# marict/nnue-vision

Hardware: AMD Instinct MI355X
Metric: NNUE training images/sec (full step: fwd+bwd+clip+SGD) (higher is better)
Workload: dtype f32; 1 GPU; c2: NNUE 32x32 grid 10x10x8 F=800 -> 1024/128/32 -> 10, batch 512/GPU, SGD m0.9 wd2e-4 clip1.0; global_batch=512, parallelism=dp1, launch=hipGraph, steps_per_graph=26, max_active_features=453

## Files before the change

nnue-vision_amd/csrc/classifier_kernels.hip:

```cpp
#include <type_traits>
#include <cstdlib>
#include <cstring>

#include "common.h"
#include "small_wgrad.h"

namespace {

using f32x4 = __attribute__((ext_vector_type(4))) float;

__device__ __forceinline__ float act_fn(float z, float clip) {
  const float r = z <= 0.0f ? 0.0f : z;
  return (clip > 0.0f && r > clip) ? clip : r;
}
__device__ __forceinline__ float gate_fn(float d, float h, float clip) {
  if (clip > 0.0f) return (h > 0.0f && h < clip) ? d : 0.0f;
  return h <= 0.0f ? 0.0f : d;
}

__device__ __forceinline__ float l0_at(const float* __restrict__ xr, int k, int half, int pairwise) {
  if (!pairwise) return xr[k];
  return k < half ? xr[k] * xr[k + half] : xr[k - half];
}

// ... 674 lines not shown
      const float* __restrict__ wr = w3 + (size_t)c * L3;
      if constexpr (VEC) {
        int k = 4 * part4;
        if (c0 == 0) {
#pragma unroll
          for (int i = 0; i < kPre3; ++i) {
            const int kk = 4 * (part4 + 4 * i);
            if (kk < L3) z = tail_dot4(w3v[i], *reinterpret_cast<const float4*>(h2s + kk), z);
          }
          k += 16 * kPre3;
        }
        for (; k < L3; k += 16) z = tail_dot4(*reinterpret_cast<const float4*>(wr + k), *reinterpret_cast<const float4*>(h2s + k), z);
      } else {
        for (int k = part4; k < L3; k += 4) z = fmaf(wr[k], h2s[k], z);
      }
    }
    z += __shfl_xor(z, 1);
    z += __shfl_xor(z, 2);
    if (c < C && part4 == 0) {
      z += (VEC && c0 == 0) ? b3v : b3[c];
      lgs[c] = z;
      logits[(size_t)b * C + c] = z;
    }
  }
  __syncthreads();
  float mx = -INFINITY, se = 0.f;
  if (C <= 64) {
    const int lane = tid & 63;
    const float v[1] = {lane < C ? lgs[lane] : -INFINITY};
    float m1[1], s1[1];
    ce_wave_stats<1>(v, lane < C, m1, s1);
    mx = m1[0];
    se = s1[0];
  } else {
    for (int c = tid; c < C; c += NT) mx = fmaxf(mx, lgs[c]);
    mx = block_reduce_nt<NT>(mx, true, red);
    for (int c = tid; c < C; c += NT) se += expf(lgs[c] - mx);
    se = block_reduce_nt<NT>(se, false, red);
  }
  const bool ok = y >= 0 && y < C;
  if (tid == 0) sample_loss[b] = ok ? nnue_ce_sample_loss(mx, lgs[y], se) : 0.0f;
  const float inv = 1.0f / se;
  __syncthreads();
  for (int c = tid; c < C; c += NT) {
    const float g = ok ? ce_dlogit(lgs[c], mx, inv, c == y, scale_over_b) : 0.0f;
    lgs[c] = g;
    d_logits[(size_t)b * C + c] = g;
  }
  __syncthreads();
  for (int j0 = 0; j0 < L3; j0 += 32) {
    const int j = j0 + (tid & 31), cp = tid >> 5;
    part_s[cp][tid & 31] = j < L3 ? dz2_slice<S>(lgs, w3 + j, cp, C, L3) : 0.0f;
    __syncthreads();
    if (cp == 0 && j < L3) {
      float q[S];
#pragma unroll
      for (int i = 0; i < S; ++i) q[i] = part_s[i][tid];
      const float v = gate_fn(slice_tree<S>(q), h2s[j], clip);
      dz2s[j] = v;
      d_z2[(size_t)b * L3 + j] = v;
    }
    __syncthreads();
  }
  for (int k = tid; k < L2; k += NT) {
    float s = 0.f;
    int j = 0;
    for (; j + 16 <= L3; j += 16) {
      float w[16];
#pragma unroll
      for (int u = 0; u < 16; ++u) w[u] = w2[(size_t)(j + u) * L2 + k];
#pragma unroll
      for (int u = 0; u < 16; ++u) s = fmaf(dz2s[j + u], w[u], s);
    }
    for (; j < L3; ++j) s = fmaf(dz2s[j], w2[(size_t)j * L2 + k], s);
    const float v = gate_fn(s, h1s[k], clip);
    d_z1[(size_t)b * L2 + k] = v;
    if (d_z1_g) d_z1_g[(size_t)g * L2 + k] = v;
  }
  __syncthreads();
}

constexpr int kTdxRows = 16, kTdxThreads = 512, kTdxMaxC = 64;

template <int S>
__device__ __forceinline__ float dz2_slice_small(const float* dl, const float* w3j, int cp, int C, int L3) {
  float s0 = 0.f, s1 = 0.f, s2 = 0.f, s3 = 0.f;
  int c = cp;
  for (int m = 0, mu = C > 3 * S ? (C - 3 * S + 4 * S - 1) / (4 * S) : 0; m < mu; ++m) {
    const bool act = c + 3 * S < C;
    const int cc = act ? c : 0;
    const float f0 = fmaf(dl[cc], w3j[(size_t)cc * L3], s0), f1 = fmaf(dl[cc + S], w3j[(size_t)(cc + S) * L3], s1);
    const float f2 = fmaf(dl[cc + 2 * S], w3j[(size_t)(cc + 2 * S) * L3], s2), f3 = fmaf(dl[cc + 3 * S], w3j[(size_t)(cc + 3 * S) * L3], s3);
    s0 = act ? f0 : s0; s1 = act ? f1 : s1; s2 = act ? f2 : s2; s3 = act ? f3 : s3;
    c = act ? c + 4 * S : c;
  }
#pragma unroll
  for (int t = 0; t < 3; ++t) {
    const bool act = c + S * t < C;
    const int cc = act ? c + S * t : 0;
    const float f = fmaf(dl[cc], w3j[(size_t)cc * L3], s0);
    s0 = act ? f : s0;
  }
  return (s0 + s1) + (s2 + s3);
}

template <int L2, int L3>
__global__ __launch_bounds__(kTdxThreads) void tail_dx_train_kernel(
    const float* __restrict__ part, int ksplit, const float* __restrict__ b1, const float* __restrict__ w2,
    const float* __restrict__ b2, const float* __restrict__ w3, const float* __restrict__ b3, float clip,
    const int64_t* __restrict__ labels, float scale_over_b, int B, int C, float* __restrict__ h1, float* __restrict__ h2,
    float* __restrict__ logits, float* __restrict__ sample_loss, float* __restrict__ d_logits, float* __restrict__ d_z1,
    float* __restrict__ d_z2, const float* __restrict__ x, const float* __restrict__ w1, int L1, float* __restrict__ d_x,
    int m_tiles, int n_cg) {
  constexpr int T = kTdxRows, NT = kTdxThreads, NWAVE = NT / 64;
  constexpr int NI = T * L2 / 4 / NT;
  constexpr int NCH = L2 / (16 * kBwxKC);
  constexpr int RP = NT / 4 / L3;
  static_assert(NI >= 1 && NI * NT * 4 == T * L2 && NT % L2 == 0 && L3 % 16 == 0 && (NT / 4) % L3 == 0 && T % RP == 0,
                "tail_dx_train_kernel: unsupported layer widths");
  __shared__ float4 w2s4[L3 * L2 / 4];
  __shared__ float4 w3s4[kTdxMaxC * L3 / 4];
  __shared__ __attribute__((aligned(16))) float h1s[T][L2];
  __shared__ __attribute__((aligned(16))) float dz1s[T][L2];
  __shared__ __attribute__((aligned(16))) float h2s[T][L3];
  __shared__ float dz2s[T][L3];
  __shared__ float ps[T][4][L3];
  __shared__ float lgs[T][kTdxMaxC];
  __shared__ float b2s[L3], b3s[kTdxMaxC];
  __shared__ int64_t ys[T];
  __shared__ f32x4 xch[NWAVE][64];
  const float* w2s = reinterpret_cast<const float*>(w2s4);
  const float* w3s = reinterpret_cast<const float*>(w3s4);

  const int blk = blockIdx.x, slot = blk >> 3;
  const int mt = (slot / n_cg) * 8 + (blk & 7), cg = slot % n_cg;
  if (mt >= m_tiles) return;
  const bool writer = cg == 0;
  const int row0 = mt * T;
  const int tid = threadIdx.x;

  const int wave = __builtin_amdgcn_readfirstlane(tid >> 6);
  const int lane = tid & 63;
  const int r = lane & 15, q = lane >> 4;
  const int half = L1 / 2;
  const int hi = wave & 1;
  const int c0 = (cg * (NWAVE / 2) + (wave >> 1)) * 16, c1 = c0 + half, cm = hi ? c1 : c0;
  int orows[4];
#pragma unroll
  for (int e = 0; e < 4; ++e) orows[e] = row0 + 4 * q + e;
  float bw[NCH][kBwxKC][4];
#pragma unroll
  for (int n = 0; n < NCH; ++n) bwx_load_b_tile(bw[n], w1, n * 16 * kBwxKC, L1, L2, cm, r, q);
  float xv[4];
#pragma unroll
  for (int e = 0; e < 4; ++e) xv[e] = x[(size_t)min(orows[e], B - 1) * L1 + (hi ? c0 : c1) + r];

  constexpr int NW2 = L3 * L2 / 4 / NT;
  constexpr int NW3 = kTdxMaxC * L3 / 4 / NT;
  static_assert(NW2 >= 1 && NW2 * NT * 4 == L3 * L2 && NW3 >= 1 && NW3 * NT * 4 == kTdxMaxC * L3, "tail_dx_train_kernel: staging shape");
  float4 w2v[NW2], w3v[NW3];
#pragma unroll
  for (int i = 0; i < NW2; ++i) w2v[i] = reinterpret_cast<const float4*>(w2)[tid + NT * i];
  const int n_w3 = C * L3 / 4;
#pragma unroll
  for (int i = 0; i < NW3; ++i) w3v[i] = reinterpret_cast<const float4*>(w3)[min(tid + NT * i, n_w3 - 1)];
  const float b2v = b2[tid % L3];
  const float b3v = b3[min(tid, C - 1)];
  const int64_t yv = labels[min(row0 + (tid % T), B - 1)];
  int srow[NI], scol[NI];
  float4 z4[NI];
  const float* prow[NI];
#pragma unroll
  for (int i = 0; i < NI; ++i) {
    const int f = tid + NT * i;
    srow[i] = f / (L2 / 4);
    scol[i] = 4 * (f % (L2 / 4));
    prow[i] = part + (size_t)min(row0 + srow[i], B - 1) * L2 + scol[i];
    z4[i] = make_float4(b1[scol[i]], b1[scol[i] + 1], b1[scol[i] + 2], b1[scol[i] + 3]);
  }
  const size_t slab = (size_t)B * L2;
  auto load_batch = [&](int s0, float4 (&v)[NI][16]) {
#pragma unroll
    for (int i = 0; i < NI; ++i)
#pragma unroll
      for (int u = 0; u < 16; ++u) v[i][u] = *reinterpret_cast<const float4*>(prow[i] + (size_t)min(s0 + u, ksplit - 1) * slab);
  };
  auto sum_batch = [&](int s0, const float4 (&v)[NI][16]) {
#pragma unroll
    for (int i = 0; i < NI; ++i)
#pragma unroll
      for (int u = 0; u < 16; ++u) {
        const bool add = s0 + u < ksplit;
        z4[i].x = add ? z4[i].x + v[i][u].x : z4[i].x;
        z4[i].y = add ? z4[i].y + v[i][u].y : z4[i].y;
        z4[i].z = add ? z4[i].z + v[i][u].z : z4[i].z;
        z4[i].w = add ? z4[i].w + v[i][u].w : z4[i].w;
      }
  };
  {
    float4 v[NI][16];
    load_batch(0, v);
#pragma unroll
    for (int i = 0; i < NW2; ++i) w2s4[tid + NT * i] = w2v[i];
#pragma unroll
    for (int i = 0; i < NW3; ++i)
      if (tid + NT * i < n_w3) w3s4[tid + NT * i] = w3v[i];
    if (tid < L3) b2s[tid] = b2v;
    if (tid < C) b3s[tid] = b3v;
    if (tid < T) ys[tid] = row0 + tid < B ? yv : -1;
    sum_batch(0, v);
  }
  for (int s0 = 16; s0 < ksplit; s0 += 16) {
    float4 v[NI][16];
    load_batch(s0, v);
    sum_batch(s0, v);
  }

#pragma unroll
  for (int i = 0; i < NI; ++i) {
    float4 h;
    h.x = act_fn(z4[i].x, clip); h.y = act_fn(z4[i].y, clip); h.z = act_fn(z4[i].z, clip); h.w = act_fn(z4[i].w, clip);
    *reinterpret_cast<float4*>(&h1s[srow[i]][scol[i]]) = h;
    if (writer && row0 + srow[i] < B) *reinterpret_cast<float4*>(h1 + (size_t)(row0 + srow[i]) * L2 + scol[i]) = h;
  }
  __syncthreads();

  const int part4 = tid & 3, og = tid >> 2;
  {
    const int j = og % L3;
    float4 wf[L2 / 16];
#pragma unroll
    for (int m = 0; m < L2 / 16; ++m) wf[m] = w2s4[(j * L2 + 4 * part4 + 16 * m) / 4];
    const float bj = b2s[j];
#pragma unroll
    for (int it = 0; it < T / RP; ++it) {
      const int rr = og / L3 + RP * it;
      float z = 0.f;
#pragma unroll
      for (int m = 0; m < L2 / 16; ++m) z = tail_dot4(wf[m], *reinterpret_cast<const float4*>(&h1s[rr][4 * part4 + 16 * m]), z);
      z += lane_xor<1>(z);
      z += lane_xor<2>(z);
      if (part4 == 0) {
        const float h = act_fn(z + bj, clip);
        h2s[rr][j] = h;
        if (writer && row0 + rr < B) h2[(size_t)(row0 + rr) * L3 + j] = h;
      }
    }
  }
  __syncthreads();
  for (int o0 = 0; o0 < T * C; o0 += NT / 4) {
    const int o = o0 + og;
    const bool v = o < T * C;
    const int rr = v ? o / C : 0, c = v ? o - rr * C : 0;
    float z = 0.f;
#pragma unroll
    for (int k = 4 * part4; k < L3; k += 16)
      z = tail_dot4(*reinterpret_cast<const float4*>(w3s + c * L3 + k), *reinterpret_cast<const float4*>(&h2s[rr][k]), z);
    z = v ? z : 0.f;
    z += lane_xor<1>(z);
    z += lane_xor<2>(z);
    if (v && part4 == 0) {
      z += b3s[c];
      lgs[rr][c] = z;
      if (writer && row0 + rr < B) logits[(size_t)(row0 + rr) * C + c] = z;
    }
  }
  __syncthreads();
  {
    constexpr int RW = T / NWAVE;
    const bool in = lane < C;
    float v[RW], mx[RW], se[RW];
#pragma unroll
    for (int it = 0; it < RW; ++it) v[it] = in ? lgs[wave + NWAVE * it][lane] : -INFINITY;
    ce_wave_stats_fast<RW>(v, in, mx, se);
#pragma unroll
    for (int it = 0; it < RW; ++it) {
      const int rr = wave + NWAVE * it;
      const int64_t y = ys[rr];
      const bool ok = y >= 0 && y < C;
      const float zy = ok ? lgs[rr][y] : 0.f;
      if (writer && lane == 0 && row0 + rr < B) sample_loss[row0 + rr] = ok ? nnue_ce_sample_loss(mx[it], zy, se[it]) : 0.0f;
      const float inv = 1.0f / se[it];
      if (in) {
        const float g = ok ? ce_dlogit(v[it], mx[it], inv, lane == y, scale_over_b) : 0.0f;
        lgs[rr][lane] = g;
        if (writer && row0 + rr < B) d_logits[(size_t)(row0 + rr) * C + lane] = g;
      }
    }
  }
  __syncthreads();
#pragma unroll
  for (int it = 0; it < T * 4 * L3 / NT; ++it) {
    const int i = tid + NT * it;
    const int j = i % L3, cp = (i / L3) & 3, rr = i / (4 * L3);
    ps[rr][cp][j] = dz2_slice_small<4>(lgs[rr], w3s + j, cp, C, L3);
  }
  __syncthreads();
#pragma unroll
  for (int it = 0; it < (T * L3 + NT - 1) / NT; ++it) {
    const int i = tid + NT * it, rr = i / L3, j = i % L3;
    if (i < T * L3) {
      float qv[4] = {ps[rr][0][j], ps[rr][1][j], ps[rr][2][j], ps[rr][3][j]};
      const float v = gate_fn(slice_tree<4>(qv), h2s[rr][j], clip);
      dz2s[rr][j] = v;
      if (writer && row0 + rr < B) d_z2[(size_t)(row0 + rr) * L3 + j] = v;
    }
  }
  __syncthreads();
  {
    const int k = tid % L2;
    float wc[L3];
#pragma unroll
    for (int j = 0; j < L3; ++j) wc[j] = w2s[j * L2 + k];
#pragma unroll
    for (int it = 0; it < T * L2 / NT; ++it) {
      const int rr = tid / L2 + (NT / L2) * it;
      float s = 0.f;
#pragma unroll
      for (int j = 0; j < L3; ++j) s = fmaf(dz2s[rr][j], wc[j], s);
      const float v = gate_fn(s, h1s[rr][k], clip);
      dz1s[rr][k] = v;
      if (writer && row0 + rr < B) d_z1[(size_t)(row0 + rr) * L2 + k] = v;
    }
  }
  __syncthreads();
  {
    const bool row_ok = row0 + r < B;
    f32x4 acc = (f32x4){0.f, 0.f, 0.f, 0.f};
#pragma unroll
    for (int n = 0; n < NCH; ++n) {
      BwxChunk ch;
      bwx_load_a(ch, &dz1s[r][0], row_ok, n * 16 * kBwxKC, L2, q);
      bwx_mma_tile(ch.a, bw[n], acc);
    }
    xch[wave][lane] = acc;
    __syncthreads();
    const f32x4 other = xch[wave ^ 1][lane];
#pragma unroll
    for (int e = 0; e < 4; ++e) {
      const int orow = orows[e];
      if (orow >= B) continue;
      float* __restrict__ o = d_x + (size_t)orow * L1;
      if (hi) o[c1 + r] = other[e] * xv[e];
      else o[c0 + r] = fmaf(acc[e], xv[e], other[e]);
    }
  }
}

struct ClsPlan {
  bool fwd_mfma, bww_mfma, bwx_mfma;
  int fwd_ksplit;
  int bww_ksplit, bww_klen;
};

int bucket_tiles(int B, int K) { return (B + 15) / 16 + K; }

bool tail_dx_supported(int B, int L1, int L2, int L3, int C, int K, int pairwise) {
  return B > 0 && K == 1 && pairwise && L1 > 0 && L1 % 128 == 0 && C >= 1 && C <= kTdxMaxC && L2 == 128 && L3 == 32;
}

ClsPlan make_plan(int B, int L1, int L2, int pairwise, int K = 1) {
  ClsPlan p{};
  p.fwd_mfma = (L1 % 32 == 0) && (L2 % 16 == 0);
  p.fwd_ksplit = 1;
  if (p.fwd_mfma) {
    const int tiles = (K > 1 ? bucket_tiles(B, K) : (B + 15) / 16) * ((L2 + 63) / 64);
    int ks = 1;
    while (tiles * ks < 1024 && L1 % (ks * 2 * 16) == 0 && L1 / (ks * 2) >= 64) ks *= 2;
    if (pairwise && ks == 1) ks = 2;
    static const int force_ks = [] { const char* e = getenv("NNUE_CLS_FWD_KSPLIT"); return e ? atoi(e) : 0; }();
    if (force_ks >= 2 && (force_ks & (force_ks - 1)) == 0 && L1 % (force_ks * 16) == 0 && L1 / force_ks >= 32) ks = force_ks;
    p.fwd_ksplit = ks;
  }
  p.bww_mfma = (L1 % 64 == 0) && (L2 % 32 == 0);
  p.bww_ksplit = 1;
  p.bww_klen = B;
  if (p.bww_mfma && K > 1) {
    const int tiles = (L2 / 32) * (L1 / 64);
    int ks = 1;
    while (tiles * ks < 512 && B / (ks * 2) >= 64) ks *= 2;
    p.bww_ksplit = ks;
    p.bww_klen = (((B + ks - 1) / ks) + 15) / 16 * 16;
  } else if (p.bww_mfma) {
    const int tiles = (L2 / 32) * (L1 / 64);
    int ks = 1;
    while (tiles * ks < 1024 && B / (ks * 2) >= 32) ks *= 2;
    p.bww_ksplit = ks;
    p.bww_klen = ((B + ks - 1) / ks + 3) / 4 * 4;
  }
  p.bwx_mfma = (L1 % 32 == 0) && (L2 % 16 == 0);
  return p;
}

int64_t plan_scratch_floats(const ClsPlan& p, int B, int L1, int L2, int L3, int K = 1) {
  const int64_t fwd = (int64_t)p.fwd_ksplit * B * L2;
  const int64_t bwd = (int64_t)B * L2 + (int64_t)B * L3 + (p.bww_ksplit > 1 ? (int64_t)p.bww_ksplit * K * L2 * L1 : 0);
  return (fwd > bwd ? fwd : bwd) + 64;
}

#include "bucket_group.h"

constexpr int kGroupThreads = 1024;
__global__ __launch_bounds__(kGroupThreads) void bucket_group_kernel(GroupArgs ga) {
  __shared__ int lds[kGroupLdsInts];
  bucket_group_body<kGroupThreads>(ga, lds);
}

Buckets no_buckets() { return Buckets{1, nullptr, nullptr, nullptr, nullptr, 0}; }

int buckets_from(const nnue_buckets* c, int B, Buckets* out, const char* who) {
  *out = no_buckets();
  if (!c || c->K <= 1) return NNUE_OK;
  NNUE_REQUIRE(c->K <= kMaxBuckets, NNUE_E_SHAPE, "%s: %d layer stacks (at most %d)", who, c->K, kMaxBuckets);
  NNUE_REQUIRE(c->bucket && c->rows && c->tile_bucket && c->seg, NNUE_E_ARG, "%s: null bucket pointer", who);
  NNUE_REQUIRE(c->tiles == bucket_tiles(B, c->K), NNUE_E_SHAPE, "%s: bucket grouping was made for another batch (tiles %d, expected %d)", who,
               c->tiles, bucket_tiles(B, c->K));
  *out = Buckets{c->K, c->bucket, c->rows, c->tile_bucket, c->seg, c->tiles};
  return NNUE_OK;
}

}

namespace {

int forward_impl(const float* x, int pairwise, const float* w1, const float* b1, const float* w2, const float* b2, const float* w3,
                 const float* b3, float clip, int B, int L1, int L2, int L3, int C, float* h1, float* h2, float* logits, void* scratch,
                 int64_t scratch_bytes, const Buckets& bk, nnue_stream_t stream) {
  NNUE_REQUIRE(x && w1 && b1 && w2 && b2 && w3 && b3 && h1 && h2 && logits && scratch, NNUE_E_ARG,
               "nnue_classifier_forward: null pointer");
// ... 90 lines not shown
}

extern "C" int nnue_bucket_tile_count(int B, int K) { return (B > 0 && K > 0) ? bucket_tiles(B, K) : 0; }

extern "C" int nnue_bucket_group(const int32_t* n, int B, int P, int K, int32_t* bucket, int32_t* rows, int32_t* tile_bucket,
                                 int32_t* seg, nnue_stream_t stream) {
  NNUE_REQUIRE(n && bucket && rows && tile_bucket && seg, NNUE_E_ARG, "nnue_bucket_group: null pointer");
  NNUE_REQUIRE(B > 0 && P >= 0 && K >= 1, NNUE_E_ARG, "nnue_bucket_group: B=%d P=%d K=%d out of range", B, P, K);
  NNUE_REQUIRE(K <= kMaxBuckets, NNUE_E_SHAPE, "nnue_bucket_group: %d layer stacks (at most %d)", K, kMaxBuckets);
  hipLaunchKernelGGL(bucket_group_kernel, dim3(1), dim3(kGroupThreads), 0, static_cast<hipStream_t>(stream),
                     GroupArgs{n, B, P, K, bucket, rows, tile_bucket, seg, bucket_tiles(B, K)});
  return nnue_launch_status("nnue_bucket_group");
}

extern "C" int nnue_classifier_forward(const float* x, int pairwise, const float* w1, const float* b1, const float* w2,
                                       const float* b2, const float* w3, const float* b3, float clip, int B, int L1,
                                       int L2, int L3, int C, float* h1, float* h2, float* logits, void* scratch,
                                       int64_t scratch_bytes, nnue_stream_t stream) {
  return forward_impl(x, pairwise, w1, b1, w2, b2, w3, b3, clip, B, L1, L2, L3, C, h1, h2, logits, scratch, scratch_bytes, no_buckets(),
                      stream);
}

extern "C" int nnue_classifier_forward_bucketed(const float* x, int pairwise, const float* w1, const float* b1, const float* w2,
                                                const float* b2, const float* w3, const float* b3, float clip, int B, int L1, int L2,
                                                int L3, int C, float* h1, float* h2, float* logits, void* scratch,
                                                int64_t scratch_bytes, const nnue_buckets* buckets, nnue_stream_t stream) {
  Buckets bk;
  const int rc = buckets_from(buckets, B, &bk, "nnue_classifier_forward_bucketed");
  if (rc != NNUE_OK) return rc;
  return forward_impl(x, pairwise, w1, b1, w2, b2, w3, b3, clip, B, L1, L2, L3, C, h1, h2, logits, scratch, scratch_bytes, bk, stream);
}

extern "C" int nnue_classifier_backward(const float* x, int pairwise, const float* w1, const float* w2, const float* w3,
                                        float clip, const float* h1, const float* h2, const float* d_logits, int B, int L1,
                                        int L2, int L3, int C, float* d_x, float* d_w1, float* d_b1, float* d_w2,
                                        float* d_b2, float* d_w3, float* d_b3, void* scratch, int64_t scratch_bytes,
                                        nnue_stream_t stream) {
  return backward_impl(x, pairwise, w1, w2, w3, clip, h1, h2, d_logits, B, L1, L2, L3, C, d_x, d_w1, d_b1, d_w2, d_b2, d_w3, d_b3, scratch,
                       scratch_bytes, no_buckets(), stream);
}

extern "C" int nnue_classifier_backward_bucketed(const float* x, int pairwise, const float* w1, const float* w2, const float* w3,
                                                 float clip, const float* h1, const float* h2, const float* d_logits, int B, int L1,
                                                 int L2, int L3, int C, float* d_x, float* d_w1, float* d_b1, float* d_w2, float* d_b2,
                                                 float* d_w3, float* d_b3, void* scratch, int64_t scratch_bytes,
                                                 const nnue_buckets* buckets, nnue_stream_t stream) {
  Buckets bk;
  const int rc = buckets_from(buckets, B, &bk, "nnue_classifier_backward_bucketed");
  if (rc != NNUE_OK) return rc;
  return backward_impl(x, pairwise, w1, w2, w3, clip, h1, h2, d_logits, B, L1, L2, L3, C, d_x, d_w1, d_b1, d_w2, d_b2, d_w3, d_b3, scratch,
                       scratch_bytes, bk, stream);
}

__global__ __launch_bounds__(256) void l1_backward_x_small_wgrad(const float* __restrict__ x, int pairwise, const float* __restrict__ w1,
                                                                 const float* __restrict__ d_z1, int B, int L1, int L2,
                                                                 float* __restrict__ d_x, int x_blocks, SmallWgrad a) {
  if ((int)blockIdx.x < x_blocks) l1_backward_x_body(x, pairwise, w1, d_z1, B, L1, L2, d_x, blockIdx.x, a.bk);
  else {
    __shared__ float red[1024];
    small_wgrad_body(a, (int)blockIdx.x - x_blocks, red);
  }
}

namespace {
struct TrainLayout {
  int64_t part, d_z1, d_z2, d_logits, slabs, d_z1_g, x_g, total;
};
TrainLayout train_layout(const ClsPlan& p, int B, int L1, int L2, int L3, int C, int K = 1) {
  TrainLayout t{};
  int64_t off = 0;
  auto take = [&](int64_t n) { const int64_t o = off; off += nnue_round_up(n, 4); return o; };
  const int64_t ext = (L1 % 64 == 0) ? L1 / 64 : 0;
  t.part = take((p.fwd_ksplit > ext ? (int64_t)p.fwd_ksplit : ext) * B * L2);
  t.d_z1 = take((int64_t)B * L2);
  t.d_z2 = take((int64_t)B * L3);
  t.d_logits = take((int64_t)B * C);
  t.slabs = take(p.bww_ksplit > 1 ? (int64_t)p.bww_ksplit * K * L2 * L1 : 0);
  const int64_t grows = K > 1 ? (int64_t)bucket_tiles(B, K) * 16 : 0;
  t.d_z1_g = take(grows * L2);
  t.x_g = take(grows * L1);
  t.total = off + 4;
  return t;
}

int train_step_impl(const float* x, int pairwise, const float* w1, const float* b1, const float* w2, const float* b2, const float* w3,
                    const float* b3, float clip, const int64_t* labels, float grad_scale, int B, int L1, int L2, int L3, int C, float* h1,
                    float* h2, float* logits, float* sample_loss, float* loss, float* d_x, float* d_w1, float* d_b1, float* d_w2,
                    float* d_b2, float* d_w3, float* d_b3, void* scratch, int64_t scratch_bytes, int phases, const Buckets& bk,
                    nnue_stream_t stream) {
  NNUE_REQUIRE(x && w1 && b1 && w2 && b2 && w3 && b3 && labels && h1 && h2 && logits && sample_loss && loss && scratch,
               NNUE_E_ARG, "nnue_classifier_train_step: null pointer");
  const bool fuse_tail = phases == 123;
  if (fuse_tail) phases = 59;
  NNUE_REQUIRE(phases >= 1 && phases <= 63 && (phases & 3) && (phases & 20) != 20 && (!(phases & 32) || (phases & 19) == 19), NNUE_E_ARG,
               "nnue_classifier_train_step: phases = 1 (activations + d_x) | 2 (weight gradients + loss) [| 4: first-layer weight product beside "
               "d_x] [| 8: layer-1 slabs already at the start of scratch] [| 16 (not with 4): d_w1 comes from nnue_ftm_backward] [| 32 (with 1, 2 "
               "and 16): the small gradients and the mean loss ride in nnue_ftm_backward's launch as well] [| 64 (only as 123 = 59 + 64): the "
               "per-sample tail runs in the d_x launch]");
  const bool ext_dw1 = (phases & 16) != 0;
  const bool ext_small = (phases & 32) != 0;
  const bool ext_slabs = (phases & 8) != 0;
  const int K = bk.K;
  NNUE_REQUIRE(K == 1 || !ext_slabs, NNUE_E_ARG,
               "nnue_classifier_train_step: phases bit 8 (layer-1 slabs formed in the FeatureTransformer forward's epilogue) exists for one layer stack only");
  NNUE_REQUIRE(K == 1 || !ext_dw1 || (pairwise && L1 % 4 == 0), NNUE_E_SHAPE,
               "nnue_classifier_train_step: phases bit 16 with K > 1 needs the pairwise block and L1 %% 4 == 0");
  NNUE_REQUIRE(!ext_slabs || (pairwise && L1 % 64 == 0), NNUE_E_SHAPE,
               "nnue_classifier_train_step: phases bit 8 needs the pairwise block and L1 %% 64 == 0 (got L1=%d)", L1);
  NNUE_REQUIRE(d_w1 && d_b1 && d_w2 && d_b2 && d_w3 && d_b3, NNUE_E_ARG, "nnue_classifier_train_step: null gradient pointer");
  NNUE_REQUIRE(B > 0 && L1 > 0 && L2 > 0 && L3 > 0 && C > 0, NNUE_E_ARG,
               "nnue_classifier_train_step: B=%d L1=%d L2=%d L3=%d C=%d must be positive", B, L1, L2, L3, C);
  NNUE_REQUIRE(!pairwise || L1 % 2 == 0, NNUE_E_SHAPE, "nnue_classifier_train_step: pairwise needs an even L1 (got %d)", L1);
  const int64_t tail_lds = ((int64_t)L2 + 2 * L3 + C + 8) * 4;
  NNUE_REQUIRE(tail_lds <= 64 * 1024, NNUE_E_SHAPE, "nnue_classifier_train_step: L2+2*L3+C too large for the LDS tail");
  const ClsPlan p = make_plan(B, L1, L2, pairwise, K);
  const TrainLayout t = train_layout(p, B, L1, L2, L3, C, K);
  NNUE_REQUIRE(scratch_bytes >= t.total * (int64_t)sizeof(float), NNUE_E_SCRATCH,
               "nnue_classifier_train_step: scratch %lld < %lld bytes", (long long)scratch_bytes, (long long)(t.total * 4));
  NNUE_REQUIRE(nnue_aligned16(x) && nnue_aligned16(w1) && nnue_aligned16(scratch) && nnue_aligned16(d_w1) && nnue_aligned16(h1) &&
                   nnue_aligned16(h2),
               NNUE_E_ARG, "nnue_classifier_train_step: pointers must be 16-byte aligned");
  hipStream_t s = static_cast<hipStream_t>(stream);
  float* base = static_cast<float*>(scratch);
  float *part = base + t.part, *d_z1 = base + t.d_z1, *d_z2 = base + t.d_z2, *d_logits = base + t.d_logits, *slabs = base + t.slabs;
  const bool grouped = K > 1 && ext_dw1;
  float* d_z1_g = grouped ? base + t.d_z1_g : nullptr;
  float* x_g = grouped ? base + t.x_g : nullptr;
  const int tail_grid = grouped ? bk.tiles * 16 : B;
  const bool slab_pass = p.bww_mfma && p.bww_ksplit > 1;
  const int m_tiles = bk.rows ? bk.tiles : (B + 15) / 16;
  const bool early_bww = (phases & 4) && p.bwx_mfma && p.bww_mfma && d_x != nullptr;
  const int tail_slabs = ext_slabs ? L1 / 64 : p.fwd_ksplit;
  const int wgrad_blocks = small_wgrad_tiles(L2, L3, C) * K + 1;
  const long long count = (long long)K * L2 * L1;
  const int slab_blocks = slab_pass && !ext_dw1 ? (int)((count / 4 + 255) / 256) : 0;
  const SmallWgrad sw{d_logits, d_z2, d_z1, h1, h2, B, L2, L3, C, d_w3, d_b3, d_w2, d_b2, d_b1, sample_loss, loss, wgrad_blocks,
                      slabs, slab_pass && !ext_dw1 ? p.bww_ksplit : 0, count, d_w1, bk, p.bww_klen};
  const bool wgrad_rides = (phases & 3) == 3 && ext_dw1 && p.bwx_mfma && d_x != nullptr;
  NNUE_REQUIRE(!ext_small || wgrad_rides, NNUE_E_SHAPE,
               "nnue_classifier_train_step: phases bit 32 needs the d_x launch the small gradients otherwise ride in (MFMA shapes, d_x requested)");
  NNUE_REQUIRE(!fuse_tail || tail_dx_supported(B, L1, L2, L3, C, K, pairwise), NNUE_E_SHAPE,
               "nnue_classifier_train_step: phases 123 (tail inside the d_x launch) needs nnue_classifier_train_fused_tail_supported "
               "(B=%d L1=%d L2=%d L3=%d C=%d K=%d pairwise=%d)", B, L1, L2, L3, C, K, pairwise);
  NNUE_REQUIRE(!fuse_tail || (nnue_aligned16(w2) && nnue_aligned16(w3)), NNUE_E_ARG,
               "nnue_classifier_train_step: phases 123 needs 16-byte aligned w2 and w3");
  if (fuse_tail) {
    const int n_cg = L1 / 32 / (kTdxThreads / 128);
    hipLaunchKernelGGL((tail_dx_train_kernel<128, 32>), dim3((m_tiles + 7) / 8 * 8 * n_cg), dim3(kTdxThreads), 0, s, part, L1 / 64, b1, w2, b2,
                       w3, b3, clip, labels, grad_scale / (float)B, B, C, h1, h2, logits, sample_loss, d_logits, d_z1, d_z2, x, w1, L1, d_x,
                       m_tiles, n_cg);
    return nnue_launch_status("nnue_classifier_train_step");
  }
  if (phases & 1) {
    if (ext_slabs) {
    } else if (p.fwd_mfma) {
      const long long waves = (long long)m_tiles * ((L2 + 63) / 64) * p.fwd_ksplit;
      hipLaunchKernelGGL(l1_forward_mfma, dim3((unsigned)((waves + 3) / 4)), dim3(256), 0, s, x, pairwise, w1, B, L1, L2, p.fwd_ksplit, part, bk);
    } else {
      const long long waves = (long long)B * L2;
      hipLaunchKernelGGL(l1_forward_simple, dim3((unsigned)((waves + 3) / 4)), dim3(256), 0, s, x, pairwise, w1, B, L1, L2, part, bk);
    }
    const bool vec = L2 % 4 == 0 && L3 % 4 == 0 && nnue_aligned16(w2) && nnue_aligned16(w3);
#define NNUE_TAIL(NT, V)                                                                                                                  \
  hipLaunchKernelGGL((tail_train_kernel<NT, V>), dim3(tail_grid), dim3(NT), (size_t)tail_lds, s, part, tail_slabs, b1, w2, b2, w3, b3, clip, \
                     labels, grad_scale / (float)B, B, L2, L3, C, h1, h2, logits, sample_loss, d_logits, d_z1, d_z2, bk, x, L1, x_g, d_z1_g)
    if (C > 256) { if (vec) NNUE_TAIL(512, true); else NNUE_TAIL(512, false); }
    else { if (vec) NNUE_TAIL(128, true); else NNUE_TAIL(128, false); }
#undef NNUE_TAIL
    if (d_x) {
      if (p.bwx_mfma && early_bww) {
        const long long xw = (long long)m_tiles * (L1 / 32), ww = (long long)K * (L2 / 32) * (L1 / 64) * p.bww_ksplit;
        const int w_blocks = (int)((ww + 3) / 4);
        hipLaunchKernelGGL(l1_backward_xw_mfma, dim3((unsigned)(w_blocks + (xw + 3) / 4)), dim3(256), 0, s, x, pairwise, w1, d_z1, B, L1, L2,
                           d_x, w_blocks, p.bww_ksplit, p.bww_klen, slab_pass ? slabs : d_w1, bk);
      } else if (wgrad_rides) {
        const long long waves = (long long)m_tiles * (L1 / 32);
        const int x_blocks = (int)((waves + 3) / 4);
#ifdef NNUE_ABLATIONS
        static const int skip_small = [] { const char* e = getenv("NNUE_CLS_ABL_SKIP_SMALL"); return e ? atoi(e) : 0; }();
#else
        constexpr int skip_small = 0;
#endif
        hipLaunchKernelGGL(l1_backward_x_small_wgrad, dim3((unsigned)(x_blocks + ((skip_small || ext_small) ? 0 : wgrad_blocks))), dim3(256), 0, s, x, pairwise, w1,
                           (const float*)d_z1, B, L1, L2, d_x, x_blocks, sw);
      } else if (p.bwx_mfma) {
        const long long waves = (long long)m_tiles * (L1 / 32);
        hipLaunchKernelGGL(l1_backward_x_mfma, dim3((unsigned)((waves + 3) / 4)), dim3(256), 0, s, x, pairwise, w1, d_z1, B, L1, L2, d_x, bk);
      } else {
        const int cols = pairwise ? L1 / 2 : L1;
        hipLaunchKernelGGL(l1_backward_x_simple, dim3(B, (cols + 255) / 256), dim3(256), 0, s, x, pairwise, w1, d_z1, B, L1, L2, d_x, bk);
      }
    }
  }
  if (wgrad_rides) return nnue_launch_status("nnue_classifier_train_step");
  if (phases & 2) {
    if (early_bww || ext_dw1) {
    } else if (p.bww_mfma) {
      const long long waves = (long long)K * (L2 / 32) * (L1 / 64) * p.bww_ksplit;
      hipLaunchKernelGGL(l1_backward_w_mfma, dim3((unsigned)((waves + 3) / 4)), dim3(256), 0, s, x, pairwise, d_z1, B, L1, L2, p.bww_ksplit,
                         p.bww_klen, slab_pass ? slabs : d_w1, bk);
    } else {
      hipLaunchKernelGGL(l1_backward_w_simple, dim3(K * L2, (L1 + 255) / 256), dim3(256), 0, s, x, pairwise, d_z1, B, L1, L2, d_w1, bk);
    }
    hipLaunchKernelGGL(small_wgrad_kernel, dim3(wgrad_blocks + slab_blocks), dim3(256), 0, s, sw);
  }
  return nnue_launch_status("nnue_classifier_train_step");
}
}

extern "C" int64_t nnue_classifier_train_scratch(int B, int L1, int L2, int L3, int C) {
  return nnue_classifier_train_scratch_bucketed(B, L1, L2, L3, C, 1);
}

extern "C" int64_t nnue_classifier_train_scratch_bucketed(int B, int L1, int L2, int L3, int C, int K) {
  if (B <= 0 || L1 <= 0 || L2 <= 0 || L3 <= 0 || C <= 0 || K <= 0) return 0;
  const int64_t a = train_layout(make_plan(B, L1, L2, 0, K), B, L1, L2, L3, C, K).total;
  const int64_t b = train_layout(make_plan(B, L1, L2, 1, K), B, L1, L2, L3, C, K).total;
  return (a > b ? a : b) * (int64_t)sizeof(float);
}

extern "C" int nnue_classifier_train_fused_tail_supported(int B, int L1, int L2, int L3, int C, int K, int pairwise) {
  return tail_dx_supported(B, L1, L2, L3, C, K, pairwise) ? 1 : 0;
}

extern "C" int64_t nnue_classifier_train_dz1_offset(int B, int L1, int L2, int L3, int C, int pairwise) {
  if (B <= 0 || L1 <= 0 || L2 <= 0 || L3 <= 0 || C <= 0) return -1;
  return train_layout(make_plan(B, L1, L2, pairwise), B, L1, L2, L3, C).d_z1 * (int64_t)sizeof(float);
}

extern "C" int64_t nnue_classifier_train_dz1_grouped_offset(int B, int L1, int L2, int L3, int C, int K) {
  if (B <= 0 || L1 <= 0 || L2 <= 0 || L3 <= 0 || C <= 0 || K <= 1 || K > kMaxBuckets) return -1;
  return train_layout(make_plan(B, L1, L2, 1, K), B, L1, L2, L3, C, K).d_z1_g * (int64_t)sizeof(float);
}

extern "C" int64_t nnue_classifier_train_x_grouped_offset(int B, int L1, int L2, int L3, int C, int K) {
  if (B <= 0 || L1 <= 0 || L2 <= 0 || L3 <= 0 || C <= 0 || K <= 1 || K > kMaxBuckets) return -1;
  return train_layout(make_plan(B, L1, L2, 1, K), B, L1, L2, L3, C, K).x_g * (int64_t)sizeof(float);
}

extern "C" int nnue_classifier_train_rider(int pairwise, int B, int L1, int L2, int L3, int C, const float* h1, const float* h2,
                                           const float* sample_loss, float* loss, float* d_b1, float* d_w2, float* d_b2, float* d_w3,
                                           float* d_b3, void* scratch, int64_t scratch_bytes, const nnue_buckets* buckets,
                                           nnue_cls_rider* out) {
  NNUE_REQUIRE(h1 && h2 && sample_loss && loss && d_b1 && d_w2 && d_b2 && d_w3 && d_b3 && scratch && out, NNUE_E_ARG,
               "nnue_classifier_train_rider: null pointer");
  NNUE_REQUIRE(B > 0 && L1 > 0 && L2 > 0 && L3 > 0 && C > 0, NNUE_E_ARG, "nnue_classifier_train_rider: sizes must be positive");
  Buckets bk;
  const int rc = buckets_from(buckets, B, &bk, "nnue_classifier_train_rider");
  if (rc != NNUE_OK) return rc;
  const ClsPlan p = make_plan(B, L1, L2, pairwise, bk.K);
  const TrainLayout t = train_layout(p, B, L1, L2, L3, C, bk.K);
  NNUE_REQUIRE(scratch_bytes >= t.total * (int64_t)sizeof(float), NNUE_E_SCRATCH, "nnue_classifier_train_rider: scratch %lld < %lld bytes",
               (long long)scratch_bytes, (long long)(t.total * 4));
  float* base = static_cast<float*>(scratch);
  const int wgrad_blocks = small_wgrad_tiles(L2, L3, C) * bk.K + 1;
  const SmallWgrad sw{base + t.d_logits, base + t.d_z2, base + t.d_z1, h1, h2, B, L2, L3, C, d_w3, d_b3, d_w2, d_b2, d_b1, sample_loss, loss,
                      wgrad_blocks, nullptr, 0, (long long)bk.K * L2 * L1, nullptr, bk, p.bww_klen};
  static_assert(sizeof(SmallWgrad) <= sizeof(nnue_cls_rider), "nnue_cls_rider is too small");
  memset(out, 0, sizeof(*out));
  memcpy(out, &sw, sizeof(sw));
  return NNUE_OK;
}

extern "C" int nnue_classifier_train_step(const float* x, int pairwise, const float* w1, const float* b1, const float* w2,
                                          const float* b2, const float* w3, const float* b3, float clip,
                                          const int64_t* labels, float grad_scale, int B, int L1, int L2, int L3, int C,
                                          float* h1, float* h2, float* logits, float* sample_loss, float* loss, float* d_x,
                                          float* d_w1, float* d_b1, float* d_w2, float* d_b2, float* d_w3, float* d_b3,
                                          void* scratch, int64_t scratch_bytes, int phases, nnue_stream_t stream) {
  return train_step_impl(x, pairwise, w1, b1, w2, b2, w3, b3, clip, labels, grad_scale, B, L1, L2, L3, C, h1, h2, logits, sample_loss, loss,
                         d_x, d_w1, d_b1, d_w2, d_b2, d_w3, d_b3, scratch, scratch_bytes, phases, no_buckets(), stream);
}

extern "C" int nnue_classifier_train_step_bucketed(const float* x, int pairwise, const float* w1, const float* b1, const float* w2,
                                                   const float* b2, const float* w3, const float* b3, float clip, const int64_t* labels,
                                                   float grad_scale, int B, int L1, int L2, int L3, int C, float* h1, float* h2,
                                                   float* logits, float* sample_loss, float* loss, float* d_x, float* d_w1, float* d_b1,
                                                   float* d_w2, float* d_b2, float* d_w3, float* d_b3, void* scratch,
                                                   int64_t scratch_bytes, int phases, const nnue_buckets* buckets, nnue_stream_t stream) {
  Buckets bk;
  const int rc = buckets_from(buckets, B, &bk, "nnue_classifier_train_step_bucketed");
  if (rc != NNUE_OK) return rc;
  return train_step_impl(x, pairwise, w1, b1, w2, b2, w3, b3, clip, labels, grad_scale, B, L1, L2, L3, C, h1, h2, logits, sample_loss, loss,
                         d_x, d_w1, d_b1, d_w2, d_b2, d_w3, d_b3, scratch, scratch_bytes, phases, bk, stream);
}
```

Measured before the change: 8.004 million images/sec.

## Compute fused tail layer products with fp32 MFMA and register-held weight fragments

Rewrites the forward h2/logits and backward dz2/dz1 small matmuls in the fused tail kernel to use 16x16x4 fp32 MFMA, with w2/w3 fragments loaded straight into registers instead of staged through LDS. Scalar dot products with lane shuffles go away, and the partial sums are reduced through a small shared buffer. A DX template flag lets the same tiled tail replace the generic tail kernel on the non-fused path when it is supported. The change also adds ablation clock probes behind a compile flag, and it ties the kernel to L2=128 and L3=32.

```diff
diff --git a/nnue-vision_amd/csrc/classifier_kernels.hip b/nnue-vision_amd/csrc/classifier_kernels.hip
--- a/nnue-vision_amd/csrc/classifier_kernels.hip
+++ b/nnue-vision_amd/csrc/classifier_kernels.hip
@@ -780,55 +780,69 @@
 
 constexpr int kTdxRows = 16, kTdxThreads = 512, kTdxMaxC = 64;
 
-template <int S>
-__device__ __forceinline__ float dz2_slice_small(const float* dl, const float* w3j, int cp, int C, int L3) {
-  float s0 = 0.f, s1 = 0.f, s2 = 0.f, s3 = 0.f;
-  int c = cp;
-  for (int m = 0, mu = C > 3 * S ? (C - 3 * S + 4 * S - 1) / (4 * S) : 0; m < mu; ++m) {
-    const bool act = c + 3 * S < C;
-    const int cc = act ? c : 0;
-    const float f0 = fmaf(dl[cc], w3j[(size_t)cc * L3], s0), f1 = fmaf(dl[cc + S], w3j[(size_t)(cc + S) * L3], s1);
-    const float f2 = fmaf(dl[cc + 2 * S], w3j[(size_t)(cc + 2 * S) * L3], s2), f3 = fmaf(dl[cc + 3 * S], w3j[(size_t)(cc + 3 * S) * L3], s3);
-    s0 = act ? f0 : s0; s1 = act ? f1 : s1; s2 = act ? f2 : s2; s3 = act ? f3 : s3;
-    c = act ? c + 4 * S : c;
-  }
-#pragma unroll
-  for (int t = 0; t < 3; ++t) {
-    const bool act = c + S * t < C;
-    const int cc = act ? c + S * t : 0;
-    const float f = fmaf(dl[cc], w3j[(size_t)cc * L3], s0);
-    s0 = act ? f : s0;
-  }
-  return (s0 + s1) + (s2 + s3);
-}
+#ifdef NNUE_ABLATIONS
+constexpr int kTdxClocks = 10;
+struct TdxAbl { long long* clocks; };
+#define NNUE_TDX_ABL_PARAM , TdxAbl abl
+#define NNUE_TDX_CLOCK(i) do { if (abl.clocks && threadIdx.x == 0) abl.clocks[(size_t)blockIdx.x * kTdxClocks + (i)] = clock64(); } while (0)
+#else
+#define NNUE_TDX_ABL_PARAM
+#define NNUE_TDX_CLOCK(i) do { } while (0)
+#endif
+
+struct TailFrags {
+  float w2f[8];
+  float w2b[8];
+  float w3f[8];
+  float b3v;
+};
 
 template <int L2, int L3>
+__device__ __forceinline__ void tail_load_frags(TailFrags& f, const float* __restrict__ w2, const float* __restrict__ w3,
+                                                const float* __restrict__ b3, int C, int wave, int r, int q) {
+  static_assert(L2 == 128 && L3 == 32, "tail_load_frags: the wave roles are laid out for 128 / 32");
+  const int t = wave & 1, kq = wave >> 1, kh = (wave >> 1) & 1;
+  const bool lg = wave < 4;
+#pragma unroll
+  for (int i = 0; i < 8; ++i) {
+    const int k = 16 * (i >> 2) + 4 * q + (i & 3);
+    f.w2f[i] = w2[(16 * t + r) * L2 + 32 * kq + k];
+    f.w2b[i] = w2[k * L2 + 16 * wave + r];
+    const int cls = lg ? 16 * wave + r : 32 * kh + k, unit = lg ? k : 16 * t + r;
+    f.w3f[i] = w3[min(cls, C - 1) * L3 + unit];
+  }
+  f.b3v = b3[min(16 * (wave & 3) + r, C - 1)];
+}
+
+__device__ __forceinline__ f32x4 tail_mma4(const float4& a, float b0, float b1, float b2, float b3, f32x4 acc) {
+  acc = __builtin_amdgcn_mfma_f32_16x16x4f32(a.x, b0, acc, 0, 0, 0);
+  acc = __builtin_amdgcn_mfma_f32_16x16x4f32(a.y, b1, acc, 0, 0, 0);
+  acc = __builtin_amdgcn_mfma_f32_16x16x4f32(a.z, b2, acc, 0, 0, 0);
+  acc = __builtin_amdgcn_mfma_f32_16x16x4f32(a.w, b3, acc, 0, 0, 0);
+  return acc;
+}
+
+template <int L2, int L3, bool DX, bool SKIP = false>
 __global__ __launch_bounds__(kTdxThreads) void tail_dx_train_kernel(
     const float* __restrict__ part, int ksplit, const float* __restrict__ b1, const float* __restrict__ w2,
     const float* __restrict__ b2, const float* __restrict__ w3, const float* __restrict__ b3, float clip,
     const int64_t* __restrict__ labels, float scale_over_b, int B, int C, float* __restrict__ h1, float* __restrict__ h2,
     float* __restrict__ logits, float* __restrict__ sample_loss, float* __restrict__ d_logits, float* __restrict__ d_z1,
     float* __restrict__ d_z2, const float* __restrict__ x, const float* __restrict__ w1, int L1, float* __restrict__ d_x,
-    int m_tiles, int n_cg) {
+    int m_tiles, int n_cg NNUE_TDX_ABL_PARAM) {
   constexpr int T = kTdxRows, NT = kTdxThreads, NWAVE = NT / 64;
   constexpr int NI = T * L2 / 4 / NT;
   constexpr int NCH = L2 / (16 * kBwxKC);
-  constexpr int RP = NT / 4 / L3;
-  static_assert(NI >= 1 && NI * NT * 4 == T * L2 && NT % L2 == 0 && L3 % 16 == 0 && (NT / 4) % L3 == 0 && T % RP == 0,
+  static_assert(NI >= 1 && NI * NT * 4 == T * L2 && T * L3 == NT && NWAVE == 8 && T == 16,
                 "tail_dx_train_kernel: unsupported layer widths");
-  __shared__ float4 w2s4[L3 * L2 / 4];
-  __shared__ float4 w3s4[kTdxMaxC * L3 / 4];
-  __shared__ __attribute__((aligned(16))) float h1s[T][L2];
-  __shared__ __attribute__((aligned(16))) float dz1s[T][L2];
-  __shared__ __attribute__((aligned(16))) float h2s[T][L3];
-  __shared__ float dz2s[T][L3];
+  __shared__ __attribute__((aligned(16))) float h1s[T][L2 + 4];
+  __shared__ __attribute__((aligned(16))) float dz1s[T][L2 + 4];
+  __shared__ __attribute__((aligned(16))) float h2s[T][L3 + 4];
+  __shared__ __attribute__((aligned(16))) float dz2s[T][L3 + 4];
   __shared__ float ps[T][4][L3];
-  __shared__ float lgs[T][kTdxMaxC];
-  __shared__ float b2s[L3], b3s[kTdxMaxC];
+  __shared__ __attribute__((aligned(16))) float lgs[T][kTdxMaxC + 4];
   __shared__ int64_t ys[T];
-  __shared__ f32x4 xch[NWAVE][64];
-  const float* w2s = reinterpret_cast<const float*>(w2s4);
-  const float* w3s = reinterpret_cast<const float*>(w3s4);
+  __shared__ f32x4 xch[DX ? NWAVE : 1][64];
 
   const int blk = blockIdx.x, slot = blk >> 3;
   const int mt = (slot / n_cg) * 8 + (blk & 7), cg = slot % n_cg;
@@ -836,6 +850,8 @@
   const bool writer = cg == 0;
   const int row0 = mt * T;
   const int tid = threadIdx.x;
+  constexpr bool skip = SKIP;
+  NNUE_TDX_CLOCK(0);
 
   const int wave = __builtin_amdgcn_readfirstlane(tid >> 6);
   const int lane = tid & 63;
@@ -847,23 +863,17 @@
 #pragma unroll
   for (int e = 0; e < 4; ++e) orows[e] = row0 + 4 * q + e;
   float bw[NCH][kBwxKC][4];
-#pragma unroll
-  for (int n = 0; n < NCH; ++n) bwx_load_b_tile(bw[n], w1, n * 16 * kBwxKC, L1, L2, cm, r, q);
   float xv[4];
-#pragma unroll
-  for (int e = 0; e < 4; ++e) xv[e] = x[(size_t)min(orows[e], B - 1) * L1 + (hi ? c0 : c1) + r];
-
-  constexpr int NW2 = L3 * L2 / 4 / NT;
-  constexpr int NW3 = kTdxMaxC * L3 / 4 / NT;
-  static_assert(NW2 >= 1 && NW2 * NT * 4 == L3 * L2 && NW3 >= 1 && NW3 * NT * 4 == kTdxMaxC * L3, "tail_dx_train_kernel: staging shape");
-  float4 w2v[NW2], w3v[NW3];
-#pragma unroll
-  for (int i = 0; i < NW2; ++i) w2v[i] = reinterpret_cast<const float4*>(w2)[tid + NT * i];
-  const int n_w3 = C * L3 / 4;
-#pragma unroll
-  for (int i = 0; i < NW3; ++i) w3v[i] = reinterpret_cast<const float4*>(w3)[min(tid + NT * i, n_w3 - 1)];
+  if constexpr (DX) {
+#pragma unroll
+    for (int n = 0; n < NCH; ++n) bwx_load_b_tile(bw[n], w1, n * 16 * kBwxKC, L1, L2, cm, r, q);
+#pragma unroll
+    for (int e = 0; e < 4; ++e) xv[e] = x[(size_t)min(orows[e], B - 1) * L1 + (hi ? c0 : c1) + r];
+  }
+
+  TailFrags fr;
+  tail_load_frags<L2, L3>(fr, w2, w3, b3, C, wave, r, q);
   const float b2v = b2[tid % L3];
-  const float b3v = b3[min(tid, C - 1)];
   const int64_t yv = labels[min(row0 + (tid % T), B - 1)];
   int srow[NI], scol[NI];
   float4 z4[NI];
@@ -898,13 +908,6 @@
   {
     float4 v[NI][16];
     load_batch(0, v);
-#pragma unroll
-    for (int i = 0; i < NW2; ++i) w2s4[tid + NT * i] = w2v[i];
-#pragma unroll
-    for (int i = 0; i < NW3; ++i)
-      if (tid + NT * i < n_w3) w3s4[tid + NT * i] = w3v[i];
-    if (tid < L3) b2s[tid] = b2v;
-    if (tid < C) b3s[tid] = b3v;
     if (tid < T) ys[tid] = row0 + tid < B ? yv : -1;
     sum_batch(0, v);
   }
@@ -922,48 +925,60 @@
     if (writer && row0 + srow[i] < B) *reinterpret_cast<float4*>(h1 + (size_t)(row0 + srow[i]) * L2 + scol[i]) = h;
   }
   __syncthreads();
-
-  const int part4 = tid & 3, og = tid >> 2;
+  NNUE_TDX_CLOCK(1);
+
+  const f32x4 zero4 = (f32x4){0.f, 0.f, 0.f, 0.f};
+  const int orow_t = tid / L3, ounit = tid % L3;
   {
-    const int j = og % L3;
-    float4 wf[L2 / 16];
-#pragma unroll
-    for (int m = 0; m < L2 / 16; ++m) wf[m] = w2s4[(j * L2 + 4 * part4 + 16 * m) / 4];
-    const float bj = b2s[j];
-#pragma unroll
-    for (int it = 0; it < T / RP; ++it) {
-      const int rr = og / L3 + RP * it;
-      float z = 0.f;
-#pragma unroll
-      for (int m = 0; m < L2 / 16; ++m) z = tail_dot4(wf[m], *reinterpret_cast<const float4*>(&h1s[rr][4 * part4 + 16 * m]), z);
-      z += lane_xor<1>(z);
-      z += lane_xor<2>(z);
-      if (part4 == 0) {
-        const float h = act_fn(z + bj, clip);
-        h2s[rr][j] = h;
-        if (writer && row0 + rr < B) h2[(size_t)(row0 + rr) * L3 + j] = h;
+    const int t = wave & 1, kq = wave >> 1;
+    f32x4 acc = zero4;
+    if constexpr (!skip) {
+#pragma unroll
+      for (int g = 0; g < 2; ++g) {
+        const float4 a = *reinterpret_cast<const float4*>(&h1s[r][32 * kq + 16 * g + 4 * q]);
+        acc = tail_mma4(a, fr.w2f[4 * g], fr.w2f[4 * g + 1], fr.w2f[4 * g + 2], fr.w2f[4 * g + 3], acc);
       }
     }
-  }
-  __syncthreads();
-  for (int o0 = 0; o0 < T * C; o0 += NT / 4) {
-    const int o = o0 + og;
-    const bool v = o < T * C;
-    const int rr = v ? o / C : 0, c = v ? o - rr * C : 0;
-    float z = 0.f;
-#pragma unroll
-    for (int k = 4 * part4; k < L3; k += 16)
-      z = tail_dot4(*reinterpret_cast<const float4*>(w3s + c * L3 + k), *reinterpret_cast<const float4*>(&h2s[rr][k]), z);
-    z = v ? z : 0.f;
-    z += lane_xor<1>(z);
-    z += lane_xor<2>(z);
-    if (v && part4 == 0) {
-      z += b3s[c];
-      lgs[rr][c] = z;
-      if (writer && row0 + rr < B) logits[(size_t)(row0 + rr) * C + c] = z;
-    }
-  }
-  __syncthreads();
+#pragma unroll
+    for (int e = 0; e < 4; ++e) ps[4 * q + e][kq][16 * t + r] = acc[e];
+  }
+  __syncthreads();
+  NNUE_TDX_CLOCK(2);
+  {
+    float z = ps[orow_t][0][ounit];
+    z += ps[orow_t][1][ounit];
+    z += ps[orow_t][2][ounit];
+    z += ps[orow_t][3][ounit];
+    const float h = act_fn(z + b2v, clip);
+    h2s[orow_t][ounit] = h;
+    if (writer && row0 + orow_t < B) h2[(size_t)(row0 + orow_t) * L3 + ounit] = h;
+  }
+  __syncthreads();
+  NNUE_TDX_CLOCK(3);
+  if (16 * wave < C) {
+    const int n = 16 * wave + r;
+    const bool n_in = n < C;
+    f32x4 acc = zero4;
+    if constexpr (!skip) {
+#pragma unroll
+      for (int g = 0; g < 2; ++g) {
+        const float4 a = *reinterpret_cast<const float4*>(&h2s[r][16 * g + 4 * q]);
+        acc = tail_mma4(a, n_in ? fr.w3f[4 * g] : 0.f, n_in ? fr.w3f[4 * g + 1] : 0.f, n_in ? fr.w3f[4 * g + 2] : 0.f,
+                        n_in ? fr.w3f[4 * g + 3] : 0.f, acc);
+      }
+    }
+    if (n_in) {
+#pragma unroll
+      for (int e = 0; e < 4; ++e) {
+        const int rr = 4 * q + e;
+        const float z = acc[e] + fr.b3v;
+        lgs[rr][n] = z;
+        if (writer && row0 + rr < B) logits[(size_t)(row0 + rr) * C + n] = z;
+      }
+    }
+  }
+  __syncthreads();
+  NNUE_TDX_CLOCK(4);
   {
     constexpr int RW = T / NWAVE;
     const bool in = lane < C;
@@ -987,42 +1002,57 @@
     }
   }
   __syncthreads();
-#pragma unroll
-  for (int it = 0; it < T * 4 * L3 / NT; ++it) {
-    const int i = tid + NT * it;
-    const int j = i % L3, cp = (i / L3) & 3, rr = i / (4 * L3);
-    ps[rr][cp][j] = dz2_slice_small<4>(lgs[rr], w3s + j, cp, C, L3);
-  }
-  __syncthreads();
-#pragma unroll
-  for (int it = 0; it < (T * L3 + NT - 1) / NT; ++it) {
-    const int i = tid + NT * it, rr = i / L3, j = i % L3;
-    if (i < T * L3) {
-      float qv[4] = {ps[rr][0][j], ps[rr][1][j], ps[rr][2][j], ps[rr][3][j]};
-      const float v = gate_fn(slice_tree<4>(qv), h2s[rr][j], clip);
-      dz2s[rr][j] = v;
-      if (writer && row0 + rr < B) d_z2[(size_t)(row0 + rr) * L3 + j] = v;
-    }
-  }
-  __syncthreads();
+  NNUE_TDX_CLOCK(5);
+  if (wave >= 4) {
+    const int t = wave & 1, kh = (wave >> 1) & 1;
+    f32x4 acc = zero4;
+    if constexpr (!skip) {
+#pragma unroll
+      for (int g = 0; g < 2; ++g) {
+        const int cb = 32 * kh + 16 * g;
+        if (cb < C) {
+          const int c = cb + 4 * q;
+          float4 a = *reinterpret_cast<const float4*>(&lgs[r][c]);
+          a.x = c < C ? a.x : 0.f; a.y = c + 1 < C ? a.y : 0.f; a.z = c + 2 < C ? a.z : 0.f; a.w = c + 3 < C ? a.w : 0.f;
+          acc = tail_mma4(a, c < C ? fr.w3f[4 * g] : 0.f, c + 1 < C ? fr.w3f[4 * g + 1] : 0.f, c + 2 < C ? fr.w3f[4 * g + 2] : 0.f,
+                          c + 3 < C ? fr.w3f[4 * g + 3] : 0.f, acc);
+        }
+      }
+    }
+#pragma unroll
+    for (int e = 0; e < 4; ++e) ps[4 * q + e][kh][16 * t + r] = acc[e];
+  }
+  __syncthreads();
+  NNUE_TDX_CLOCK(6);
   {
-    const int k = tid % L2;
-    float wc[L3];
-#pragma unroll
-    for (int j = 0; j < L3; ++j) wc[j] = w2s[j * L2 + k];
-#pragma unroll
-    for (int it = 0; it < T * L2 / NT; ++it) {
-      const int rr = tid / L2 + (NT / L2) * it;
-      float s = 0.f;
-#pragma unroll
-      for (int j = 0; j < L3; ++j) s = fmaf(dz2s[rr][j], wc[j], s);
-      const float v = gate_fn(s, h1s[rr][k], clip);
+    const float s = ps[orow_t][0][ounit] + ps[orow_t][1][ounit];
+    const float v = gate_fn(s, h2s[orow_t][ounit], clip);
+    dz2s[orow_t][ounit] = v;
+    if (writer && row0 + orow_t < B) d_z2[(size_t)(row0 + orow_t) * L3 + ounit] = v;
+  }
+  __syncthreads();
+  NNUE_TDX_CLOCK(7);
+  {
+    f32x4 acc = zero4;
+    if constexpr (!skip) {
+#pragma unroll
+      for (int g = 0; g < 2; ++g) {
+        const float4 a = *reinterpret_cast<const float4*>(&dz2s[r][16 * g + 4 * q]);
+        acc = tail_mma4(a, fr.w2b[4 * g], fr.w2b[4 * g + 1], fr.w2b[4 * g + 2], fr.w2b[4 * g + 3], acc);
+      }
+    }
+    const int k = 16 * wave + r;
+#pragma unroll
+    for (int e = 0; e < 4; ++e) {
+      const int rr = 4 * q + e;
+      const float v = gate_fn(acc[e], h1s[rr][k], clip);
       dz1s[rr][k] = v;
       if (writer && row0 + rr < B) d_z1[(size_t)(row0 + rr) * L2 + k] = v;
     }
   }
   __syncthreads();
-  {
+  NNUE_TDX_CLOCK(8);
+  if constexpr (DX) {
     const bool row_ok = row0 + r < B;
     f32x4 acc = (f32x4){0.f, 0.f, 0.f, 0.f};
 #pragma unroll
@@ -1043,6 +1073,7 @@
       else o[c0 + r] = fmaf(acc[e], xv[e], other[e]);
     }
   }
+  NNUE_TDX_CLOCK(9);
 }
 
 struct ClsPlan {
@@ -1299,6 +1330,11 @@
   t.total = off + 4;
   return t;
 }
+
+#ifdef NNUE_ABLATIONS
+long long* g_tdx_clocks = nullptr;
+int g_tdx_clock_blocks = 0;
+#endif
 
 int train_step_impl(const float* x, int pairwise, const float* w1, const float* b1, const float* w2, const float* b2, const float* w3,
                     const float* b3, float clip, const int64_t* labels, float grad_scale, int B, int L1, int L2, int L3, int C, float* h1,
@@ -1361,11 +1397,40 @@
                "(B=%d L1=%d L2=%d L3=%d C=%d K=%d pairwise=%d)", B, L1, L2, L3, C, K, pairwise);
   NNUE_REQUIRE(!fuse_tail || (nnue_aligned16(w2) && nnue_aligned16(w3)), NNUE_E_ARG,
                "nnue_classifier_train_step: phases 123 needs 16-byte aligned w2 and w3");
+  const bool tile_tail = tail_dx_supported(B, L1, L2, L3, C, K, pairwise);
+  auto launch_tile_tail = [&](bool dx, int slabs_in) {
+    const int n_cg = dx ? L1 / 32 / (kTdxThreads / 128) : 1;
+    const int tdx_grid = (m_tiles + 7) / 8 * 8 * n_cg;
+#ifdef NNUE_ABLATIONS
+    static const int abl_skip = [] { const char* e = getenv("NNUE_CLS_ABL_SKIP_TAIL_PRODUCTS"); return e ? atoi(e) : 0; }();
+    static const int abl_clocks = [] { const char* e = getenv("NNUE_CLS_ABL_TAIL_CLOCKS"); return e ? atoi(e) : 0; }();
+    if (abl_clocks && tdx_grid > g_tdx_clock_blocks) {
+      if (g_tdx_clocks) (void)hipFree(g_tdx_clocks);
+      g_tdx_clocks = nullptr;
+      g_tdx_clock_blocks = hipMalloc(&g_tdx_clocks, (size_t)tdx_grid * kTdxClocks * sizeof(long long)) == hipSuccess ? tdx_grid : 0;
+    }
+    if (abl_clocks && g_tdx_clocks) (void)hipMemsetAsync(g_tdx_clocks, 0, (size_t)g_tdx_clock_blocks * kTdxClocks * sizeof(long long), s);
+    const TdxAbl abl{abl_clocks ? g_tdx_clocks : nullptr};
+#define NNUE_TDX_ABL_ARG , abl
+#else
+    constexpr int abl_skip = 0;
+#define NNUE_TDX_ABL_ARG
+#endif
+#define NNUE_TDX(DX, SKIP)                                                                                                                \
+  hipLaunchKernelGGL((tail_dx_train_kernel<128, 32, DX, SKIP>), dim3(tdx_grid), dim3(kTdxThreads), 0, s, part, slabs_in, b1, w2, b2, w3, b3, \
+                     clip, labels, grad_scale / (float)B, B, C, h1, h2, logits, sample_loss, d_logits, d_z1, d_z2, x, w1, L1, d_x, m_tiles, \
+                     n_cg NNUE_TDX_ABL_ARG)
+    if (abl_skip) {
+#ifdef NNUE_ABLATIONS
+      if (dx) NNUE_TDX(true, true); else NNUE_TDX(false, true);
+#endif
+    } else if (dx) NNUE_TDX(true, false);
+    else NNUE_TDX(false, false);
+#undef NNUE_TDX
+#undef NNUE_TDX_ABL_ARG
+  };
   if (fuse_tail) {
-    const int n_cg = L1 / 32 / (kTdxThreads / 128);
-    hipLaunchKernelGGL((tail_dx_train_kernel<128, 32>), dim3((m_tiles + 7) / 8 * 8 * n_cg), dim3(kTdxThreads), 0, s, part, L1 / 64, b1, w2, b2,
-                       w3, b3, clip, labels, grad_scale / (float)B, B, C, h1, h2, logits, sample_loss, d_logits, d_z1, d_z2, x, w1, L1, d_x,
-                       m_tiles, n_cg);
+    launch_tile_tail(true, L1 / 64);
     return nnue_launch_status("nnue_classifier_train_step");
   }
   if (phases & 1) {
@@ -1381,7 +1446,8 @@
 #define NNUE_TAIL(NT, V)                                                                                                                  \
   hipLaunchKernelGGL((tail_train_kernel<NT, V>), dim3(tail_grid), dim3(NT), (size_t)tail_lds, s, part, tail_slabs, b1, w2, b2, w3, b3, clip, \
                      labels, grad_scale / (float)B, B, L2, L3, C, h1, h2, logits, sample_loss, d_logits, d_z1, d_z2, bk, x, L1, x_g, d_z1_g)
-    if (C > 256) { if (vec) NNUE_TAIL(512, true); else NNUE_TAIL(512, false); }
+    if (tile_tail) launch_tile_tail(false, tail_slabs);
+    else if (C > 256) { if (vec) NNUE_TAIL(512, true); else NNUE_TAIL(512, false); }
     else { if (vec) NNUE_TAIL(128, true); else NNUE_TAIL(128, false); }
 #undef NNUE_TAIL
     if (d_x) {
@@ -1425,6 +1491,16 @@
 }
 }
 
+#ifdef NNUE_ABLATIONS
+extern "C" int nnue_cls_abl_tail_clocks(long long* out, int max_blocks) {
+  if (!g_tdx_clocks || !out) return -1;
+  const int n = g_tdx_clock_blocks < max_blocks ? g_tdx_clock_blocks : max_blocks;
+  if (hipDeviceSynchronize() != hipSuccess) return -1;
+  if (hipMemcpy(out, g_tdx_clocks, (size_t)n * kTdxClocks * sizeof(long long), hipMemcpyDeviceToHost) != hipSuccess) return -1;
+  return n;
+}
+#endif
+
 extern "C" int64_t nnue_classifier_train_scratch(int B, int L1, int L2, int L3, int C) {
   return nnue_classifier_train_scratch_bucketed(B, L1, L2, L3, C, 1);
 }
```

After: 8.285 million images/sec (median of 6 runs). 3.5% higher.
